# JamesYang007/adelie

Measured on AMD Instinct MI355X. Metric: lambda-paths/sec (100-lambda grpnet); HBM GB/s vs peak, higher is better.
Workload: dtype f64

## Files before the change

adelie_amd/csrc/kernels_filter.hip:

```cpp
#include "sweep_common.hpp"
#include <algorithm>
#include <cfloat>

namespace ahip {

namespace {

__global__ __launch_bounds__(kThreads) void shadow_build_kernel(const double* __restrict__ X, int64_t ld, int64_t n,
                                                                float* __restrict__ Xs, int64_t lds, double* __restrict__ err,
                                                                double* __restrict__ nrm, int32_t* __restrict__ bad) {
    const int64_t j = blockIdx.x;
    const int tid = threadIdx.x;
    const double* col = X + j * ld;
    float* dst = Xs + j * lds;
    double e2 = 0, n2 = 0;
    bool any_bad = false;
    for (int64_t i = tid; i < lds; i += kThreads) {
        float f = 0.f;
        if (i < n) {
            const double x = col[i];
            const bool ok = fabs(x) <= double(FLT_MAX);
            any_bad = any_bad || !ok;
            f = ok ? float(x) : 0.f;
            const double d = x - double(f);
            e2 = fma(d, d, e2);
            n2 = fma(double(f), double(f), n2);
        }
        dst[i] = f;
    }
    __shared__ double red[2][kThreads / 64];
    const int lane = tid & 63, wv = tid >> 6;
    e2 = wave_sum(e2);
    n2 = wave_sum(n2);
    if (lane == 0) { red[0][wv] = e2; red[1][wv] = n2; }
    __syncthreads();
    if (tid == 0) {
        double a = 0, b = 0;
        for (int w = 0; w < kThreads / 64; ++w) { a += red[0][w]; b += red[1][w]; }
        err[j] = sqrt(a) * (1.0 + 1e-9);
        nrm[j] = sqrt(b) * (1.0 + 1e-9);
    }
    if (any_bad) atomicOr(bad, 1);
}

__global__ __launch_bounds__(kThreads) void shadow_build_q15_kernel(const double* __restrict__ X, int64_t ld, int64_t n,
                                                                    int16_t* __restrict__ Xq, int64_t lds,
                                                                    double* __restrict__ scale, double* __restrict__ err,
                                                                    double* __restrict__ nrm, int32_t* __restrict__ bad) {
#pragma clang fp contract(off)
    const int64_t j = blockIdx.x;
    const int tid = threadIdx.x, lane = tid & 63, wv = tid >> 6;
    const double* col = X + j * ld;
    int16_t* dst = Xq + j * lds;
    __shared__ double red[2][kThreads / 64];
    double m = 0;
    bool any_bad = false;
    for (int64_t i = tid; i < n; i += kThreads) {
        const double a = fabs(col[i]);
        const bool ok = a <= DBL_MAX;
        any_bad = any_bad || !ok;
        m = ok ? fmax(m, a) : m;
    }
#pragma unroll
    for (int off = 32; off > 0; off >>= 1) m = fmax(m, __shfl_down(m, off, 64));
    if (lane == 0) red[0][wv] = m;
    __syncthreads();
    m = red[0][0];
#pragma unroll
    for (int w = 1; w < kThreads / 64; ++w) m = fmax(m, red[0][w]);
    __syncthreads();
    double inv = m > 0 ? 32767.0 / m : 0.0;
    double sc = m / 32767.0;
    if (!(inv <= DBL_MAX) || !(sc >= DBL_MIN)) { inv = 0; sc = 0; }
    double e2 = 0, q2 = 0;
    for (int64_t i = tid; i < lds; i += kThreads) {
        int q = 0;
        if (i < n && sc > 0) {
            double x = col[i];
            if (!(fabs(x) <= DBL_MAX)) x = 0;
            const double t = fmin(fmax(rint(__dmul_rn(x, inv)), -32767.0), 32767.0);
            q = int(t);
            const double d = (x - __dmul_rn(sc, t)) / sc;
            e2 = fma(d, d, e2);
            q2 = fma(t, t, q2);
        }
        dst[i] = int16_t(q);
    }
    e2 = wave_sum(e2);
    q2 = wave_sum(q2);
    if (lane == 0) { red[0][wv] = e2; red[1][wv] = q2; }
    __syncthreads();
    if (tid == 0) {
        double a = 0, b = 0;
        for (int w = 0; w < kThreads / 64; ++w) { a += red[0][w]; b += red[1][w]; }
        scale[j] = sc;
        err[j] = (sc > 0 ? sc * sqrt(a) : sqrt(double(n)) * m) * (1.0 + 1e-9);
        nrm[j] = sc * sqrt(b) * (1.0 + 1e-9);
    }
    if (any_bad) atomicOr(bad, 1);
}

__global__ __launch_bounds__(kThreads) void vmul_sq_kernel(const double* __restrict__ a, const double* __restrict__ b,
                                                           double* __restrict__ out, int64_t n, double* __restrict__ part) {
    double acc = 0;
    for (int64_t i = int64_t(blockIdx.x) * blockDim.x + threadIdx.x; i < n; i += int64_t(gridDim.x) * blockDim.x) {
        const double x = a[i] * b[i];
        out[i] = x;
        acc = fma(x, x, acc);
    }
    __shared__ double red[kThreads / 64];
    const int lane = threadIdx.x & 63, wv = threadIdx.x >> 6;
    acc = wave_sum(acc);
    if (lane == 0) red[wv] = acc;
    __syncthreads();
    if (threadIdx.x == 0) {
        double s = 0;
        for (int w = 0; w < kThreads / 64; ++w) s += red[w];
        part[blockIdx.x] = s;
    }
}

__device__ __forceinline__ void shadow_guard(double exact, double approx, int64_t j, const double* __restrict__ err,
                                             const double* __restrict__ nrm, double fp_term, const double* __restrict__ vnorm,
                                             int32_t* __restrict__ flags) {
    const double bound = (err[j] + fp_term * nrm[j]) * vnorm[0];
    if (!(fabs(exact - approx) <= bound)) atomicOr(flags, 2);
}

template <int VEC>
__device__ __forceinline__ double list_column_sum(const DenseAcc<double>& X, const double* __restrict__ v, int64_t j, int64_t r0,
                                                  int64_t r1, double* red) {
    const int tid = threadIdx.x;
    const double* cp = X.colptr(j);
    double acc = 0;
    const int64_t body_end = r0 + ((r1 - r0) / VEC) * VEC;
#pragma unroll 8
    for (int64_t i = r0 + int64_t(tid) * VEC; i < body_end; i += int64_t(kThreads) * VEC) {
        const Pack<double, VEC> vv = load_vec<double, VEC>(v + i);
        const Pack<double, VEC> xx = X.template load<VEC>(cp, i, j);
#pragma unroll
        for (int e = 0; e < VEC; ++e) acc = fma(xx.v[e], vv.v[e], acc);
    }
    for (int64_t i = body_end + tid; i < r1; i += kThreads) acc = fma(X.template load<1>(cp, i, j).v[0], v[i], acc);
    const int lane = tid & 63, wv = tid >> 6;
    const double ws = wave_sum(acc);
    if (lane == 0) red[wv] = ws;
    __syncthreads();
    double s = 0;
    if (tid == 0) {
#pragma unroll
        for (int w = 0; w < kThreads / 64; ++w) s += red[w];
    }
    return s;
}

struct ShadowF32 {
    using elem = float;
    using vec = f4_t;
    static constexpr int CB = kShadowCB, VEC = kShadowVec, kUnroll = 2;
    static constexpr bool kScaled = false;
    static __device__ __forceinline__ double row(vec x, int e) { return double(x[e]); }
};
typedef int i4_t __attribute__((ext_vector_type(4)));
struct ShadowQ15 {
    using elem = int16_t;
    using vec = i4_t;
    static constexpr int CB = kShadowCB16, VEC = kShadowVec16, kUnroll = 1;
    static constexpr bool kScaled = true;
    static_assert(VEC == 8, "one 16-byte load holds 8 rows");
    static __device__ __forceinline__ double row(vec x, int e) {
        return e % 2 ? double(x[e / 2] >> 16) : double(int(int16_t(x[e / 2])));
    }
};

template <int XVEC>
__device__ __forceinline__ void exact_part(const DenseAcc<double>& X, const double* __restrict__ v, int64_t n,
                                           const int32_t* __restrict__ xa, int64_t na, const int32_t* __restrict__ xb,
                                           int64_t nb, int64_t x_rows_per_split, double* __restrict__ stage, double* red) {
    const int64_t ne = na + nb;
    const int64_t c = int64_t(blockIdx.x) % ne;
    const int64_t xsplit = int64_t(blockIdx.x) / ne;
    const int64_t j = c < na ? xa[c] : xb[c - na];
    const int64_t xr0 = xsplit * x_rows_per_split;
    const double s = list_column_sum<XVEC>(X, v, j, xr0, min(n, xr0 + x_rows_per_split), red);
    if (threadIdx.x == 0) stage[xsplit * ne + c] = s;
}

template <class Kind, int XVEC>
__global__ __launch_bounds__(kThreads) void shadow_sweep_kernel(const typename Kind::elem* __restrict__ Xs, int64_t ld,
                                                                const double* __restrict__ scale, const double* __restrict__ v,
                                                                double* __restrict__ out, int64_t n, int64_t ncols,
                                                                int64_t blocks_c, int64_t rows_per_split, int nsplit,
                                                                const double* __restrict__ sub_scale,
                                                                const double* __restrict__ sub_vec, DenseAcc<double> X,
                                                                const int32_t* __restrict__ xa, int64_t na,
                                                                const int32_t* __restrict__ xb, int64_t nb,
                                                                int64_t x_rows_per_split, int x_nsplit, double* __restrict__ stage) {
    constexpr int CB = Kind::CB, VEC = Kind::VEC;
    const int tid = threadIdx.x;
    const int64_t n_exact = (na + nb) * x_nsplit;
    __shared__ double red[kThreads / 64][CB];
    if (int64_t(blockIdx.x) < n_exact) {
        exact_part<XVEC>(X, v, n, xa, na, xb, nb, x_rows_per_split, stage, &red[0][0]);
        return;
    }
    const int64_t b = int64_t(blockIdx.x) - n_exact;
    const int64_t cb = b % blocks_c;
    const int split = int(b / blocks_c);
    const int64_t r0 = int64_t(split) * rows_per_split;
    const int64_t r1 = min(n, r0 + rows_per_split);
    const typename Kind::elem* cp[CB];
#pragma unroll
    for (int k = 0; k < CB; ++k) {
        int64_t c = cb * CB + k;
        if (c >= ncols) c = ncols - 1;
        cp[k] = Xs + c * ld;
    }
    double acc[CB];
#pragma unroll
    for (int k = 0; k < CB; ++k) acc[k] = 0;
    const int64_t body_end = r0 + ((r1 - r0) / VEC) * VEC;
#pragma unroll Kind::kUnroll
    for (int64_t i = r0 + int64_t(tid) * VEC; i < body_end; i += int64_t(kThreads) * VEC) {
        d2_t vv[VEC / 2];
#pragma unroll
        for (int e = 0; e < VEC / 2; ++e) vv[e] = *reinterpret_cast<const d2_t*>(v + i + 2 * e);
        typename Kind::vec xx[CB];
#pragma unroll
        for (int k = 0; k < CB; ++k) xx[k] = __builtin_nontemporal_load(reinterpret_cast<const typename Kind::vec*>(cp[k] + i));
#pragma unroll
        for (int k = 0; k < CB; ++k) {
#pragma unroll
            for (int e = 0; e < VEC; ++e) acc[k] = fma(Kind::row(xx[k], e), vv[e / 2][e % 2], acc[k]);
        }
    }
    for (int64_t i = body_end + tid; i < r1; i += kThreads) {
        const double vi = v[i];
#pragma unroll
        for (int k = 0; k < CB; ++k) acc[k] = fma(double(cp[k][i]), vi, acc[k]);
    }
    panel_epilogue<Kind::kScaled>(acc, red, cb, ncols, 0, nullptr, scale, out, split, nsplit, sub_scale, sub_vec);
}

template <int VEC>
__global__ __launch_bounds__(kThreads) void sweep_list_kernel(DenseAcc<double> X, const double* __restrict__ v,
                                                              double* __restrict__ out, double* __restrict__ part, int64_t n,
                                                              const int32_t* __restrict__ cols, int64_t max_cols,
                                                              const int32_t* __restrict__ count_dev, int64_t rows_per_split,
                                                              int nsplit, const double* __restrict__ sub_scale,
                                                              const double* __restrict__ sub_vec, const double* __restrict__ err,
                                                              const double* __restrict__ nrm, double fp_term,
                                                              const double* __restrict__ vnorm, int32_t* __restrict__ flags) {
    const int64_t c = blockIdx.x;
    const int64_t count = count_dev ? min(int64_t(count_dev[0]), max_cols) : max_cols;
    if (c >= count) return;
    const int split = blockIdx.y;
    const int64_t r0 = int64_t(split) * rows_per_split;
    const int64_t j = cols[c];
    __shared__ double red[kThreads / 64];
    double s = list_column_sum<VEC>(X, v, j, r0, min(n, r0 + rows_per_split), red);
    if (threadIdx.x == 0) {
        if (nsplit == 1) {
            s = centred(s, j, sub_scale, sub_vec);
            if (err) shadow_guard(s, out[j], j, err, nrm, fp_term, vnorm, flags);
            out[j] = s;
        } else {
            part[int64_t(split) * max_cols + c] = s;
        }
    }
}
__global__ void sweep_list_reduce_kernel(const double* __restrict__ part, double* __restrict__ out,
                                         const int32_t* __restrict__ cols, int64_t max_cols,
                                         const int32_t* __restrict__ count_dev, int nsplit, const double* __restrict__ sub_scale,
                                         const double* __restrict__ sub_vec, const double* __restrict__ err,
                                         const double* __restrict__ nrm, double fp_term, const double* __restrict__ vnorm,
                                         int32_t* __restrict__ flags) {
    const int64_t c = int64_t(blockIdx.x) * blockDim.x + threadIdx.x;
    const int64_t count = count_dev ? min(int64_t(count_dev[0]), max_cols) : max_cols;
    if (c >= count) return;
    const int64_t j = cols[c];
    double s = 0;
    for (int r = 0; r < nsplit; ++r) s += part[int64_t(r) * max_cols + c];
    s = centred(s, j, sub_scale, sub_vec);
    if (err) shadow_guard(s, out[j], j, err, nrm, fp_term, vnorm, flags);
    out[j] = s;
}

constexpr int kClassifyThreads = 1024, kClassifyRun = 6;
__global__ __launch_bounds__(kClassifyThreads) void filter_classify_kernel(
    double* __restrict__ grad, const int64_t* __restrict__ groups, const int64_t* __restrict__ group_sizes, int64_t G,
    const int32_t* __restrict__ slot, const double* __restrict__ penalty, double tstar, const double* __restrict__ err,
    const double* __restrict__ nrm, double fp_term, const double* __restrict__ sq_part, int n_part,
    const double* __restrict__ sub_scale, const double* __restrict__ sub_vec, const double* __restrict__ stage,
    const int32_t* __restrict__ xa, int64_t na, const int32_t* __restrict__ xb, int64_t nb, int x_nsplit,
    int32_t* __restrict__ list, int64_t cap, int32_t* __restrict__ meta_i, double* __restrict__ meta_d) {
    constexpr int NW = kClassifyThreads / 64, R = kClassifyRun;
    __shared__ double sred[NW];
    __shared__ int32_t wtot[NW];
    __shared__ double s_vnorm;
    __shared__ int32_t s_first[kClassifyThreads * R], s_want[kClassifyThreads * R];
    const int tid = threadIdx.x, lane = tid & 63, wv = tid >> 6;
    {
        double a = 0;
        for (int i = tid; i < n_part; i += kClassifyThreads) a += sq_part[i];
        a = wave_sum(a);
        if (lane == 0) sred[wv] = a;
        __syncthreads();
        if (tid == 0) {
            double s = 0;
            for (int w = 0; w < NW; ++w) s += sred[w];
            s_vnorm = sqrt(s) * (1.0 + 1e-6);
            meta_d[0] = s_vnorm;
            meta_d[1] = sub_scale ? sub_scale[0] : 0.0;
            meta_i[1] = 0;
            meta_i[3] = 0;
        }
        __syncthreads();
    }
    const double vnorm = s_vnorm;
    const int64_t ne = na + nb;
    for (int pass = 0; pass < 2; ++pass) {
        const int32_t* xl = pass ? xb : xa;
        const int64_t c0 = pass ? na : 0, cnt = pass ? nb : na;
        for (int64_t c = tid; c < cnt; c += kClassifyThreads) {
            const int64_t j = xl[c];
            double s = 0;
            for (int r = 0; r < x_nsplit; ++r) s += stage[int64_t(r) * ne + c0 + c];
            s = centred(s, j, sub_scale, sub_vec);
            shadow_guard(s, grad[j], j, err, nrm, fp_term, &s_vnorm, meta_i + 1);
            grad[j] = s;
        }
        __syncthreads();
    }
    int64_t run = 0;
    for (int64_t base = 0; base < G; base += int64_t(kClassifyThreads) * R) {
        int32_t k[R], sz[R];
        double thr[R], a2[R], b2[R];
        {
            int32_t sl[R];
            double pn[R];
            int64_t kk[R], ss[R];
#pragma unroll
            for (int u = 0; u < R; ++u) {
                const int64_t gu = base + int64_t(u) * kClassifyThreads + tid;
                const int64_t g = gu < G ? gu : G - 1;
                sl[u] = slot[g];
                pn[u] = penalty[g];
                kk[u] = groups[g];
                ss[u] = group_sizes[g];
            }
#pragma unroll
            for (int u = 0; u < R; ++u) {
                const bool on = base + int64_t(u) * kClassifyThreads + tid < G && sl[u] < 0 && pn[u] > 0 && ss[u] > 0;
                k[u] = int32_t(kk[u]);
                sz[u] = on ? int32_t(ss[u]) : 0;
                thr[u] = tstar * pn[u];
                a2[u] = 0;
                b2[u] = 0;
            }
        }
        int32_t longest = 0;
#pragma unroll
        for (int u = 0; u < R; ++u) longest = max(longest, sz[u]);
        for (int32_t t = 0; t < longest; ++t) {
            double x[R], e[R], m[R];
#pragma unroll
            for (int u = 0; u < R; ++u) {
                const int64_t at = t < sz[u] ? int64_t(k[u]) + t : 0;
                x[u] = grad[at];
                e[u] = err[at];
                m[u] = nrm[at];
            }
#pragma unroll
            for (int u = 0; u < R; ++u)
                if (t < sz[u]) {
                    const double b = e[u] + fp_term * m[u];
                    a2[u] = fma(x[u], x[u], a2[u]);
                    b2[u] = fma(b, b, b2[u]);
                }
        }
#pragma unroll
        for (int u = 0; u < R; ++u) {
            if (sz[u] > 0) {
                const double reach = (sqrt(a2[u]) + sqrt(b2[u]) * vnorm * (1.0 + 1e-9)) * (1.0 + 1e-9);
                if (reach < thr[u]) sz[u] = 0;
            }
            s_first[u * kClassifyThreads + tid] = k[u];
            s_want[u * kClassifyThreads + tid] = sz[u];
        }
        __syncthreads();
        int32_t mine = 0;
#pragma unroll
        for (int u = 0; u < R; ++u) mine += s_want[tid * R + u];
        int32_t inc = mine;
#pragma unroll
        for (int off = 1; off < 64; off <<= 1) {
            const int32_t y = __shfl_up(inc, off, 64);
            if (lane >= off) inc += y;
        }
        if (lane == 63) wtot[wv] = inc;
        __syncthreads();
        int32_t before = 0, total = 0;
        for (int w = 0; w < NW; ++w) {
            const int32_t t = wtot[w];
            if (w < wv) before += t;
            total += t;
        }
        int64_t at = run + before + inc - mine;
        if (mine > 0)
            for (int u = 0; u < R; ++u) {
                const int32_t first = s_first[tid * R + u], want = s_want[tid * R + u];
                for (int32_t t = 0; t < want; ++t, ++at)
                    if (at < cap) list[at] = first + t;
            }
        run += total;
        __syncthreads();
    }
    if (tid == 0) {
        meta_i[0] = int32_t(run < cap ? run : cap);
        if (run > cap) atomicOr(meta_i + 1, 1);
        meta_i[2] = int32_t(run < int64_t(0x7fffffff) ? run : int64_t(0x7fffffff));
    }
}

}

void launch_shadow_build(const DenseView<double>& X, float* Xs, int64_t lds, double* err, double* nrm, int32_t* bad,
                         hipStream_t s) {
    if (X.p <= 0) return;
    hipLaunchKernelGGL(shadow_build_kernel, dim3((unsigned)X.p), dim3(kThreads), 0, s, X.X, X.ld, X.n, Xs, lds, err, nrm, bad);
}
int64_t shadow_q15_ld(int64_t n) { return (n + kShadowPad16 - 1) / kShadowPad16 * kShadowPad16; }
void launch_shadow_build_q15(const DenseView<double>& X, int16_t* Xq, int64_t lds, double* scale, double* err, double* nrm,
                             int32_t* bad, hipStream_t s) {
    if (X.p <= 0) return;
    hipLaunchKernelGGL(shadow_build_q15_kernel, dim3((unsigned)X.p), dim3(kThreads), 0, s, X.X, X.ld, X.n, Xq, lds, scale, err, nrm,
                       bad);
}
int filter_norm_parts(int64_t n) { return int(grid1d(n, kThreads, 1024)); }

namespace {
struct ListShape {
    bool vec;
    int ns;
    int64_t rps;
};
ListShape list_shape(const DenseView<double>& X, const double* v) {
    ListShape L;
    L.vec = dense_vec_ok(X) && (reinterpret_cast<uintptr_t>(v) % 16) == 0;
    int64_t blocks_c;
    sweep_shape(X.n, X.p, L.vec ? VecOf<double>::N : 1, blocks_c, L.ns, L.rps);
    return L;
}
void launch_sweep_list(const DenseView<double>& X, const double* v, double* out, const int32_t* cols, int64_t max_cols,
                       const int32_t* count_dev, const double* sub_scale, const double* sub_vec, const ShadowView& guard,
                       const double* vnorm, int32_t* flags, double* work, hipStream_t s) {
    if (max_cols <= 0) return;
    DenseAcc<double> acc{X.X, X.ld};
    const ListShape L = list_shape(X, v);
    const auto kernel = L.vec ? sweep_list_kernel<VecOf<double>::N> : sweep_list_kernel<1>;
    hipLaunchKernelGGL(kernel, dim3((unsigned)max_cols, (unsigned)L.ns), dim3(kThreads), 0, s, acc, v, out, work, X.n, cols,
                       max_cols, count_dev, L.rps, L.ns, sub_scale, sub_vec, guard.err, guard.nrm, guard.fp_term(), vnorm, flags);
    if (L.ns > 1)
        hipLaunchKernelGGL(sweep_list_reduce_kernel, dim3((unsigned)((max_cols + 255) / 256)), dim3(256), 0, s, work, out, cols,
                           max_cols, count_dev, L.ns, sub_scale, sub_vec, guard.err, guard.nrm, guard.fp_term(), vnorm, flags);
}
int64_t shadow_work_elems(int64_t n, int64_t p) {
    int64_t blocks_c, rps;
    int ns, ns16;
    sweep_shape(n, p, kShadowVec, blocks_c, ns, rps, kShadowCB);
    sweep_shape(n, p, kShadowVec16, blocks_c, ns16, rps, kShadowCB16);
    return int64_t(std::max(ns, ns16)) * p + 16;
}
int64_t list_work_elems(int64_t n, int64_t p, int64_t max_cols) {
    int64_t blocks_c, rps;
    int ns;
    sweep_shape(n, p, 1, blocks_c, ns, rps);
    return int64_t(ns) * max_cols + 16;
}
template <class Kind, int XVEC>
void launch_shadow_sweep(const DenseView<double>& X, const ShadowView& S, const FilteredSweep& a, int64_t na, int64_t nb,
                         const ListShape& L, double* stage, hipStream_t s) {
    int64_t blocks_c, rps;
    int ns;
    sweep_shape(S.n, S.p, Kind::VEC, blocks_c, ns, rps, Kind::CB);
    hipLaunchKernelGGL((shadow_sweep_kernel<Kind, XVEC>), dim3((unsigned)((na + nb) * L.ns + blocks_c * ns)), dim3(kThreads), 0, s,
                       static_cast<const typename Kind::elem*>(S.X), S.ld, S.scale, a.v, ns == 1 ? a.grad : a.work, S.n, S.p,
                       blocks_c, rps, ns, a.sub_scale, a.sub_vec, DenseAcc<double>{X.X, X.ld}, a.screen_cols, na, a.pen0_cols, nb,
                       L.rps, L.ns, stage);
    if (ns > 1) launch_sweep_reduce<double>(a.work, a.grad, S.p, ns, 0, nullptr, a.sub_scale, a.sub_vec, s);
}
}

int64_t filtered_sweep_work_elems(int64_t n, int64_t p, int64_t n_before, int64_t cap) {
    return shadow_work_elems(n, p) + list_work_elems(n, p, std::max(n_before, cap));
}
void enqueue_filtered_sweep(const DenseView<double>& X, const ShadowView& S, const FilteredSweep& a, hipStream_t s) {
    if (S.p <= 0) return;
    const int64_t na = a.screen_cols ? a.n_screen_cols : 0, nb = a.pen0_cols ? a.n_pen0_cols : 0;
    double* stage = a.work + shadow_work_elems(S.n, S.p);
    hipLaunchKernelGGL(vmul_sq_kernel, dim3(grid1d(S.n, kThreads, 1024)), dim3(kThreads), 0, s, a.w, a.r, a.v, S.n, a.sq_part);
    const ListShape L = list_shape(X, a.v);
    constexpr int V = VecOf<double>::N;
    if (S.kind == kShadowQ15) {
        if (L.vec) launch_shadow_sweep<ShadowQ15, V>(X, S, a, na, nb, L, stage, s);
        else launch_shadow_sweep<ShadowQ15, 1>(X, S, a, na, nb, L, stage, s);
    } else {
        if (L.vec) launch_shadow_sweep<ShadowF32, V>(X, S, a, na, nb, L, stage, s);
        else launch_shadow_sweep<ShadowF32, 1>(X, S, a, na, nb, L, stage, s);
    }
    hipLaunchKernelGGL(filter_classify_kernel, dim3(1), dim3(kClassifyThreads), 0, s, a.grad, a.groups, a.group_sizes, a.G, a.slot,
                       a.penalty, a.tstar, S.err, S.nrm, S.fp_term(), a.sq_part, filter_norm_parts(S.n), a.sub_scale, a.sub_vec,
                       stage, a.screen_cols, na, a.pen0_cols, nb, L.ns, a.list, a.cap, a.meta_i, a.meta_d);
    launch_sweep_list(X, a.v, a.grad, a.list, a.cap, a.meta_i, a.sub_scale, a.sub_vec, S, a.meta_d, a.meta_i + 1, stage, s);
}

}
```

adelie_amd/csrc/sweep_shape.hpp:

```cpp
#pragma once
#include <cstdint>

namespace ahip {

constexpr int kSweepThreads = 256;
constexpr int kSweepCB = 4;
constexpr int kShadowCB = 8, kShadowVec = 4;
constexpr int kShadowCB16 = 8, kShadowVec16 = 8;
constexpr int kShadowPad16 = 64;

inline void sweep_shape(int64_t n, int64_t ncols, int vec, int64_t& blocks_c, int& nsplit, int64_t& rows_per_split,
                        int cb = kSweepCB) {
    blocks_c = (ncols + cb - 1) / cb;
    const int64_t unit = int64_t(kSweepThreads) * vec;
    const int64_t max_split = (n + unit * 4 - 1) / (unit * 4);
    int64_t want = (1024 + blocks_c - 1) / blocks_c;
    int64_t ns = want < 1 ? 1 : want;
    if (ns > max_split) ns = max_split;
    if (ns < 1) ns = 1;
    if (ns > 65535) ns = 65535;
    rows_per_split = (n + ns - 1) / ns;
    rows_per_split = ((rows_per_split + unit - 1) / unit) * unit;
    ns = (n + rows_per_split - 1) / rows_per_split;
    if (ns < 1) ns = 1;
    nsplit = int(ns);
}

}
```

Before: 4.889.

## Software-pipeline the Q15 shadow sweep body with double-buffered half panels

For the int16 shadow sweep, the body loop becomes a software pipeline. Each of two half panels of column loads is issued one trip ahead of the FMAs that consume it, with the v vector double-buffered and sched_barriers fencing each stage. Base pointers are made wave-uniform via readfirstlane so loads can use scalar addressing, and the kernel gets a waves-per-EU occupancy hint of 5. This aims to hide HBM latency in a bandwidth-bound GEMV-like sweep, at the cost of more live registers and scheduler constraints that could hurt occupancy.

```diff
diff --git a/adelie_amd/csrc/kernels_filter.hip b/adelie_amd/csrc/kernels_filter.hip
--- a/adelie_amd/csrc/kernels_filter.hip
+++ b/adelie_amd/csrc/kernels_filter.hip
@@ -158,20 +158,31 @@
     using elem = float;
     using vec = f4_t;
     static constexpr int CB = kShadowCB, VEC = kShadowVec, kUnroll = 2;
-    static constexpr bool kScaled = false;
+    static constexpr bool kScaled = false, kPipelined = false;
+    static constexpr int kMinWaves = 1;
     static __device__ __forceinline__ double row(vec x, int e) { return double(x[e]); }
 };
 typedef int i4_t __attribute__((ext_vector_type(4)));
 struct ShadowQ15 {
     using elem = int16_t;
     using vec = i4_t;
-    static constexpr int CB = kShadowCB16, VEC = kShadowVec16, kUnroll = 1;
-    static constexpr bool kScaled = true;
+    static constexpr int CB = kShadowCB16, VEC = kShadowVec16;
+    static constexpr bool kScaled = true, kPipelined = true;
+    static constexpr int kMinWaves = 5;
     static_assert(VEC == 8, "one 16-byte load holds 8 rows");
     static __device__ __forceinline__ double row(vec x, int e) {
         return e % 2 ? double(x[e / 2] >> 16) : double(int(int16_t(x[e / 2])));
     }
 };
+
+template <class T>
+using global_ptr = const __attribute__((address_space(1))) T*;
+template <class T>
+__device__ __forceinline__ global_ptr<T> uniform_ptr(const T* p) {
+    const uint64_t u = reinterpret_cast<uint64_t>(p);
+    const uint32_t l = __builtin_amdgcn_readfirstlane(uint32_t(u)), h = __builtin_amdgcn_readfirstlane(uint32_t(u >> 32));
+    return reinterpret_cast<global_ptr<T>>((uint64_t(h) << 32) | l);
+}
 
 template <int XVEC>
 __device__ __forceinline__ void exact_part(const DenseAcc<double>& X, const double* __restrict__ v, int64_t n,
@@ -187,7 +198,8 @@
 }
 
 template <class Kind, int XVEC>
-__global__ __launch_bounds__(kThreads) void shadow_sweep_kernel(const typename Kind::elem* __restrict__ Xs, int64_t ld,
+__global__ __launch_bounds__(kThreads) __attribute__((amdgpu_waves_per_eu(Kind::kMinWaves))) void shadow_sweep_kernel(
+                                                                const typename Kind::elem* __restrict__ Xs, int64_t ld,
                                                                 const double* __restrict__ scale, const double* __restrict__ v,
                                                                 double* __restrict__ out, int64_t n, int64_t ncols,
                                                                 int64_t blocks_c, int64_t rows_per_split, int nsplit,
@@ -220,18 +232,80 @@
 #pragma unroll
     for (int k = 0; k < CB; ++k) acc[k] = 0;
     const int64_t body_end = r0 + ((r1 - r0) / VEC) * VEC;
+    if constexpr (Kind::kPipelined) {
+        constexpr int H = CB / 2;
+        static_assert(CB % 2 == 0, "two half panels");
+        constexpr int64_t kStep = int64_t(kThreads) * VEC;
+        const uint32_t lo = uint32_t(tid) * VEC;
+        const int64_t full_trips = (body_end - r0) / kStep;
+        int64_t row = r0;
+        const auto xbase = [&](int k) { return uniform_ptr(cp[k] + row) + lo; };
+        const auto vbase = [&]() { return uniform_ptr(v + row) + lo; };
+        if (full_trips > 0) {
+            d2_t vc[VEC / 2], vn[VEC / 2];
+            typename Kind::vec ha[H], hb[H];
+            const auto half = [&](typename Kind::vec(&x)[H], int k0) {
+                __builtin_amdgcn_sched_barrier(0);
+#pragma unroll
+                for (int k = 0; k < H; ++k) {
+#pragma unroll
+                    for (int e = 0; e < VEC; ++e) acc[k0 + k] = fma(Kind::row(x[k], e), vc[e / 2][e % 2], acc[k0 + k]);
+                }
+                __builtin_amdgcn_sched_barrier(0);
+            };
+            const auto load_half = [&](typename Kind::vec(&x)[H], int k0) {
+#pragma unroll
+                for (int k = 0; k < H; ++k) x[k] = __builtin_nontemporal_load(reinterpret_cast<global_ptr<typename Kind::vec>>(xbase(k0 + k)));
+            };
+            const auto load_v = [&](d2_t(&vv)[VEC / 2]) {
+#pragma unroll
+                for (int e = 0; e < VEC / 2; ++e) vv[e] = *reinterpret_cast<global_ptr<d2_t>>(vbase() + 2 * e);
+            };
+            load_v(vc);
+            load_half(ha, 0);
+            load_half(hb, H);
+            for (int64_t t = 1; t < full_trips; ++t) {
+                row += kStep;
+                half(ha, 0);
+                load_half(ha, 0);
+                load_v(vn);
+                half(hb, H);
+                load_half(hb, H);
+#pragma unroll
+                for (int e = 0; e < VEC / 2; ++e) vc[e] = vn[e];
+                __builtin_amdgcn_sched_barrier(0);
+            }
+            row += kStep;
+            half(ha, 0);
+            half(hb, H);
+        }
+        if (row + int64_t(lo) < body_end) {
+            d2_t vv[VEC / 2];
+#pragma unroll
+            for (int e = 0; e < VEC / 2; ++e) vv[e] = *reinterpret_cast<global_ptr<d2_t>>(vbase() + 2 * e);
+            typename Kind::vec xx[CB];
+#pragma unroll
+            for (int k = 0; k < CB; ++k) xx[k] = __builtin_nontemporal_load(reinterpret_cast<global_ptr<typename Kind::vec>>(xbase(k)));
+#pragma unroll
+            for (int k = 0; k < CB; ++k) {
+#pragma unroll
+                for (int e = 0; e < VEC; ++e) acc[k] = fma(Kind::row(xx[k], e), vv[e / 2][e % 2], acc[k]);
+            }
+        }
+    } else {
 #pragma unroll Kind::kUnroll
-    for (int64_t i = r0 + int64_t(tid) * VEC; i < body_end; i += int64_t(kThreads) * VEC) {
-        d2_t vv[VEC / 2];
-#pragma unroll
-        for (int e = 0; e < VEC / 2; ++e) vv[e] = *reinterpret_cast<const d2_t*>(v + i + 2 * e);
-        typename Kind::vec xx[CB];
-#pragma unroll
-        for (int k = 0; k < CB; ++k) xx[k] = __builtin_nontemporal_load(reinterpret_cast<const typename Kind::vec*>(cp[k] + i));
-#pragma unroll
-        for (int k = 0; k < CB; ++k) {
-#pragma unroll
-            for (int e = 0; e < VEC; ++e) acc[k] = fma(Kind::row(xx[k], e), vv[e / 2][e % 2], acc[k]);
+        for (int64_t i = r0 + int64_t(tid) * VEC; i < body_end; i += int64_t(kThreads) * VEC) {
+            d2_t vv[VEC / 2];
+#pragma unroll
+            for (int e = 0; e < VEC / 2; ++e) vv[e] = *reinterpret_cast<const d2_t*>(v + i + 2 * e);
+            typename Kind::vec xx[CB];
+#pragma unroll
+            for (int k = 0; k < CB; ++k) xx[k] = __builtin_nontemporal_load(reinterpret_cast<const typename Kind::vec*>(cp[k] + i));
+#pragma unroll
+            for (int k = 0; k < CB; ++k) {
+#pragma unroll
+                for (int e = 0; e < VEC; ++e) acc[k] = fma(Kind::row(xx[k], e), vv[e / 2][e % 2], acc[k]);
+            }
         }
     }
     for (int64_t i = body_end + tid; i < r1; i += kThreads) {
diff --git a/adelie_amd/csrc/sweep_shape.hpp b/adelie_amd/csrc/sweep_shape.hpp
--- a/adelie_amd/csrc/sweep_shape.hpp
+++ b/adelie_amd/csrc/sweep_shape.hpp
@@ -7,6 +7,7 @@
 constexpr int kSweepCB = 4;
 constexpr int kShadowCB = 8, kShadowVec = 4;
 constexpr int kShadowCB16 = 8, kShadowVec16 = 8;
+static_assert(kShadowCB16 % 2 == 0, "the q15 body loop rotates two half panels");
 constexpr int kShadowPad16 = 64;
 
 inline void sweep_shape(int64_t n, int64_t ncols, int vec, int64_t& blocks_c, int& nsplit, int64_t& rows_per_split,
```

Measured after the change: 5.030 (median of 6 runs). +2.9%, better.
